# tangkk/audiomod

Measured on AMD Instinct MI355X. Metric: Msamples/s (48 kHz stereo) phase-vocoder pitch-shift; x real-time per GPU, higher is better.
Workload: dtype f32; 1 GPU; configs[1]: normal_pitchshift +4 st, stereo 48 kHz, fft=2048, phase-locked; streams_per_gpu=128, channels=2, block=480, hop_in=203, slices_per_channel=14190, concurrent_stream_groups=1, parallelism=stream-sharded x1, no collective, rank_sync=none

## Files before the change

audiomod_amd/csrc/pv_kernels.hip:

```cpp
#include "pv_kernels.h"
#include "pv_atan2f.h"
#include "pv_sincos.h"
#include "pv_wavefft.h"

#include <hip/hip_runtime.h>
#include <cstdlib>

namespace pv {

#ifdef PV_POISON
__device__ __forceinline__ void pv_poison_lds(char *base) {
    const uint32_t bytes = ((const __attribute__((address_space(4))) uint32_t *)__builtin_amdgcn_dispatch_ptr())[7];
    const int nt = blockDim.x * blockDim.y * blockDim.z, tid = threadIdx.x;
    for (uint32_t i = tid; i < bytes / 4; i += nt) reinterpret_cast<uint32_t *>(base)[i] = 0x7fc0dead;
    __syncthreads();
}
#define PV_POISON_LDS(base) pv_poison_lds(base)
#else
#define PV_POISON_LDS(base) ((void)0)
#endif

#define PV_PI 3.14159265358979323846

__device__ __forceinline__ float2 cmul(float2 a, float2 b) {
// ... 2678 lines not shown
            if (j < NP || tail_lane) acc4[q[j]] = write_back(j, V[j]);
        }
    } else {
#pragma unroll
        for (int j = 0; j < NS; ++j) asm volatile("" : "=v"(V[j].x), "=v"(V[j].y), "=v"(V[j].z), "=v"(V[j].w));
    }
    chain_pass_turn(l.turn, tl, lane);
    __builtin_amdgcn_s_setprio(0);
    float *__restrict__ out = c.out + (int64_t)row * c.out_stride_row + sl.k_off;
    float *__restrict__ stream = c.stream + (int64_t)row * ((int64_t)c.smask + 1);
    const bool quiet = (sl.flags & 2) != 0;
    auto emit = [&](int sidx, float y) {
        if (quiet || sidx < 0 || sidx >= sl.adv) return;
        if (c.resample) {
            stream[(uint32_t)(sl.str_pos + sidx) & (uint32_t)c.smask] = y;
        } else if (sidx < sl.kcnt) {
            out[sidx] = y;
        }
    };
#pragma unroll
    for (int j = 0; j < NS; ++j) {
        if (256 * j - R_ < sl.adv) {
            const int u = lane + 64 * j;
            const float4 d = j < 2 ? wd[j < 2 ? j : 0]
                                   : *reinterpret_cast<const float4 *>(wden + 4 * (u < fin_quads ? u : 0));
            const int s0 = 4 * u - R_;
            if (j < NP || tail_lane) {
                emit(s0, kFast ? V[j].x * d.x : V[j].x / d.x);
                emit(s0 + 1, kFast ? V[j].y * d.y : V[j].y / d.y);
                emit(s0 + 2, kFast ? V[j].z * d.z : V[j].z / d.z);
                emit(s0 + 3, kFast ? V[j].w * d.w : V[j].w / d.w);
            }
        }
    }
}

constexpr int chain_kernel_max_threads(int NC, int kPlainCore, bool kFast) {
    return NC <= 1024 ? ((kPlainCore < 0 || (kPlainCore == 3 && !kFast)) ? 768 : 1024) : 512;
}
template <int NC, int kPlainCore, int kRes, bool kFast = false>
__global__ __launch_bounds__(chain_kernel_max_threads(NC, kPlainCore, kFast)) void pv_synth_chain_kernel(
    const SynthArgs s, const ChainArgs c) {
    extern __shared__ __attribute__((aligned(16))) char smem_raw[];
    PV_POISON_LDS(reinterpret_cast<char *>(smem_raw));
    using W = WF<NC>;
    constexpr int N = 2 * NC, hs = NC, NQ = N / 4, NP = NQ / 64;
    const int wave = __builtin_amdgcn_readfirstlane(threadIdx.x >> 6), lane = threadIdx.x & 63;
    const int row = blockIdx.x, run = blockIdx.y;
    const int i_begin = c.run_off[run], i_count = c.run_off[run + 1] - i_begin;
    cf *wlds = reinterpret_cast<cf *>(smem_raw) + wave * W::LDS_CF;
    const ChainLds l = chain_carve(c, smem_raw + (size_t)c.waves * W::LDS_CF * sizeof(cf));
    chain_prologue(c, l, row, run == 0);
    const float *__restrict__ w = s.tb.window;
    const bool upper = (row % c.C) > 0;
    const int lane0 = lane;
    for (int i = wave; i < i_count; i += c.waves) {
        int lane = lane0;
        asm volatile("" : "+v"(lane));
        const ChainSlice sl = c.slices[i_begin + i];
        const int tl = sl.tl;
        const bool skip = (sl.flags & 1) && upper;
        float4 A[NP];
        if (!skip) {
            if (!PV_CHAIN_DIAG(c, 8)) synth_wave_role<NC, kPlainCore, 1, kFast>(s, row, tl, wlds, lane);
#pragma unroll
            for (int j = 0; j < NP; ++j) {
                const int i = 4 * (lane + 64 * j);
                const int e = ((i + hs) & (N - 1)) >> 1;
                const cf z0 = wlds[W::pad(e)], z1 = wlds[W::pad(e) + 1];
                const float4 ww = *reinterpret_cast<const float4 *>(w + i);
                A[j] = make_float4(z0.x * ww.x, z0.y * ww.y, z1.x * ww.z, z1.y * ww.w);
            }
        }
        const int r = sl.acc_pos & 3;
        if (r == 0) chain_slice_tail<0, NP, kRes, kFast>(c, l, sl, A, skip, row, i, lane);
        else if (r == 1) chain_slice_tail<1, NP, kRes, kFast>(c, l, sl, A, skip, row, i, lane);
        else if (r == 2) chain_slice_tail<2, NP, kRes, kFast>(c, l, sl, A, skip, row, i, lane);
        else chain_slice_tail<3, NP, kRes, kFast>(c, l, sl, A, skip, row, i, lane);
    }
    chain_epilogue(c, l, row, run == (int)gridDim.y - 1);
}

template <int kRes> __global__ __launch_bounds__(1024) void pv_frames_chain_kernel(const ChainArgs c) {
    extern __shared__ __attribute__((aligned(16))) char smem_raw[];
    PV_POISON_LDS(reinterpret_cast<char *>(smem_raw));
    const int wave = __builtin_amdgcn_readfirstlane(threadIdx.x >> 6), lane = threadIdx.x & 63;
    const int row = blockIdx.x, run = blockIdx.y;
    const int i_begin = c.run_off[run], i_count = c.run_off[run + 1] - i_begin;
    const ChainLds l = chain_carve(c, smem_raw);
    chain_prologue(c, l, row, run == 0);
    const int NQ = c.N >> 2;
    const int groups = (NQ + 511) >> 9;
    const bool upper = (row % c.C) > 0;
    for (int i = wave; i < i_count; i += c.waves) {
        const ChainSlice sl = c.slices[i_begin + i];
        const int tl = sl.tl;
        const bool skip = (sl.flags & 1) && upper;
        ChainPrefetch pf;
        chain_prefetch(c, sl, row, lane, pf);
        const int fslot = (int)((c.t0 + tl) & (int64_t)(c.FR - 1));
        const float4 *__restrict__ fr =
            reinterpret_cast<const float4 *>(c.frames + ((int64_t)row * c.FR + fslot) * c.N);
        auto load_group = [&](int g, float4 (&A)[8]) {
#pragma unroll
            for (int j = 0; j < 8; ++j) {
                const int u = lane + 64 * (8 * g + j);
                A[j] = (u < NQ && !skip) ? fr[u] : make_float4(0.f, 0.f, 0.f, 0.f);
            }
        };
        float4 A[8];
        load_group(0, A);
        chain_wait_turn(l.turn, i);
        if (!skip) {
            float4 prevR = make_float4(0.f, 0.f, 0.f, 0.f);
            for (int g = 0; g < groups; ++g) {
                if (g > 0) load_group(g, A);
                chain_add_dispatch<8>(l.acc, c.AR, sl.acc_pos, NQ, lane, 8 * g, A, prevR, g == groups - 1);
            }
            wave_sync();
        }
        chain_finish_slice<kRes>(c, l, sl, pf, row, i, lane);
    }
    chain_epilogue(c, l, row, run == (int)gridDim.y - 1);
}

size_t chain_lds_bytes(const ChainArgs &a, int nc_wave) {
    const size_t per_wave = nc_wave == 256    ? WF<256>::LDS_CF * sizeof(cf)
                            : nc_wave == 512  ? WF<512>::LDS_CF * sizeof(cf)
                            : nc_wave == 1024 ? WF<1024>::LDS_CF * sizeof(cf)
                            : nc_wave == 2048 ? WF<2048>::LDS_CF * sizeof(cf) : 0;
    return (size_t)a.waves * per_wave + chain_shared_bytes(a);
}

template <int NC, int kPlainCore> static void launch_synth_chain_res(const SynthArgs &s, const ChainArgs &c, hipStream_t st) {
    const size_t lds = chain_lds_bytes(c, NC);
    const bool use_fast = kPlainCore >= 0 && c.fast;
    const int kMaxThreads = use_fast ? chain_kernel_max_threads(NC, kPlainCore, true) : chain_kernel_max_threads(NC, kPlainCore, false);
    if (64 * c.waves > kMaxThreads) {
        fprintf(stderr, "audiomod_pv: fused kernel launch of %d waves exceeds its bounds (%d threads): not launched\n", c.waves, kMaxThreads);
        return;
    }
    const dim3 grid(c.rows, c.runs), block(64 * c.waves);
    static unsigned long long m0 = 0, m1 = 0, f0 = 0, f1 = 0;
    if constexpr (kPlainCore >= 0) {
        if (c.fast) {
            if (!c.resample) {
                allow_big_lds_dev(pv_synth_chain_kernel<NC, kPlainCore, 0, true>, f0);
                hipLaunchKernelGGL((pv_synth_chain_kernel<NC, kPlainCore, 0, true>), grid, block, lds, st, s, c);
            } else {
                allow_big_lds_dev(pv_synth_chain_kernel<NC, kPlainCore, 1, true>, f1);
                hipLaunchKernelGGL((pv_synth_chain_kernel<NC, kPlainCore, 1, true>), grid, block, lds, st, s, c);
            }
            return;
        }
    }
    if (!c.resample) {
        allow_big_lds_dev(pv_synth_chain_kernel<NC, kPlainCore, 0>, m0);
        hipLaunchKernelGGL((pv_synth_chain_kernel<NC, kPlainCore, 0>), grid, block, lds, st, s, c);
    } else {
        allow_big_lds_dev(pv_synth_chain_kernel<NC, kPlainCore, 1>, m1);
        hipLaunchKernelGGL((pv_synth_chain_kernel<NC, kPlainCore, 1>), grid, block, lds, st, s, c);
    }
}
bool synth_chain_has_fast(const SynthArgs &s) {
    const bool plain = !s.do_freq_comp && s.voc_band_len < 0 && !s.robotic && !s.passthru && !s.whisper &&
                       !synth_generic_only() && s.coremode >= 0 && s.coremode <= 2;
    const bool fc_locked = s.do_freq_comp && s.voc_band_len < 0 && !s.robotic && !s.passthru && !s.whisper &&
                           !synth_generic_only() && s.coremode == 1;
    return (s.tb.nc == 1024 && (plain || fc_locked)) || (s.tb.nc == 2048 && plain) ||
           ((s.tb.nc == 512 || s.tb.nc == 256) && plain);
}

void launch_synth_chain(const SynthArgs &s, const ChainArgs &c, hipStream_t st) {
    const bool plain = !s.do_freq_comp && s.voc_band_len < 0 && !s.robotic && !s.passthru && !s.whisper &&
                       !synth_generic_only() && s.coremode >= 0 && s.coremode <= 2;
    const bool fc_locked = s.do_freq_comp && s.voc_band_len < 0 && !s.robotic && !s.passthru && !s.whisper &&
                           !synth_generic_only() && s.coremode == 1;
    if (s.tb.nc == 256) {
        if (plain && s.coremode == 1) launch_synth_chain_res<256, 1>(s, c, st);
        else if (plain && s.coremode == 0) launch_synth_chain_res<256, 0>(s, c, st);
        else if (plain) launch_synth_chain_res<256, 2>(s, c, st);
        else launch_synth_chain_res<256, -1>(s, c, st);
    } else if (s.tb.nc == 512) {
        if (plain && s.coremode == 1) launch_synth_chain_res<512, 1>(s, c, st);
        else if (plain && s.coremode == 0) launch_synth_chain_res<512, 0>(s, c, st);
        else if (plain) launch_synth_chain_res<512, 2>(s, c, st);
        else launch_synth_chain_res<512, -1>(s, c, st);
    } else if (s.tb.nc == 1024) {
        if (fc_locked) launch_synth_chain_res<1024, 3>(s, c, st);
        else if (plain && s.coremode == 1) launch_synth_chain_res<1024, 1>(s, c, st);
        else if (plain && s.coremode == 0) launch_synth_chain_res<1024, 0>(s, c, st);
        else if (plain) launch_synth_chain_res<1024, 2>(s, c, st);
        else launch_synth_chain_res<1024, -1>(s, c, st);
    } else {
        if (plain && s.coremode == 1) launch_synth_chain_res<2048, 1>(s, c, st);
        else if (plain && s.coremode == 0) launch_synth_chain_res<2048, 0>(s, c, st);
        else if (plain) launch_synth_chain_res<2048, 2>(s, c, st);
        else launch_synth_chain_res<2048, -1>(s, c, st);
    }
}

void launch_frames_chain(const ChainArgs &c, hipStream_t st) {
    const size_t lds = chain_lds_bytes(c, 0);
    const dim3 grid(c.rows, c.runs), block(64 * c.waves);
    static unsigned long long m0 = 0, m1 = 0;
    if (!c.resample) {
        allow_big_lds_dev(pv_frames_chain_kernel<0>, m0);
        hipLaunchKernelGGL(pv_frames_chain_kernel<0>, grid, block, lds, st, c);
    } else {
        allow_big_lds_dev(pv_frames_chain_kernel<1>, m1);
        hipLaunchKernelGGL(pv_frames_chain_kernel<1>, grid, block, lds, st, c);
    }
}

constexpr int kResRows = 4;

template <int kRes>
__global__ __launch_bounds__(kTileOut) void pv_resample_kernel(const ResArgs a) {
    extern __shared__ __attribute__((aligned(16))) char smem_raw[];
    PV_POISON_LDS(reinterpret_cast<char *>(smem_raw));
    constexpr int NR = kResRows;
    float4 *tab4 = reinterpret_cast<float4 *>(smem_raw);
    float *stab = reinterpret_cast<float *>(smem_raw);
    float *xs = reinterpret_cast<float *>(smem_raw + a.tab_bytes);
    const int nt = blockDim.x, tid = threadIdx.x;
    const ResTile tile = a.tiles[blockIdx.x];
    const int row0 = blockIdx.y * NR, NF = a.filt_len;
    const int nr = a.rows - row0 < NR ? a.rows - row0 : NR;
    uint2 oe = make_uint2(0u, 0u);
    if (tid < tile.kcnt) oe = a.otab[(int64_t)blockIdx.x * kTileOut + tid];
    float xv[NR][2];
#pragma unroll
    for (int r = 0; r < NR; ++r) {
        const float *__restrict__ st = a.stream + (int64_t)(r < nr ? row0 + r : row0) * ((int64_t)a.smask + 1);
#pragma unroll
        for (int h = 0; h < 2; ++h) {
            const int i = tid + h * kTileOut;
            const int64_t n = tile.n_lo + i;
            xv[r][h] = (i < tile.n_cnt && n >= 0) ? st[(uint32_t)n & (uint32_t)a.smask] : 0.f;
        }
    }
    if (kRes == 2) {
        const int cnt = a.oversample * (NF + 1);
        for (int i = tid; i < cnt; i += nt) tab4[i] = a.tab4[i];
    } else {
        for (int i = tid; i < a.sinc_len; i += nt) stab[i] = a.sinc[i];
    }
#pragma unroll
    for (int r = 0; r < NR; ++r) {
#pragma unroll
        for (int h = 0; h < 2; ++h) {
            const int i = tid + h * kTileOut;
            if (i < tile.n_cnt) xs[r * a.lds_floats + i] = xv[r][h];
        }
    }
    for (int i = tid + 2 * kTileOut; i < tile.n_cnt; i += nt)
        for (int r = 0; r < nr; ++r) {
            const int64_t n = tile.n_lo + i;
            const float *__restrict__ st = a.stream + (int64_t)(row0 + r) * ((int64_t)a.smask + 1);
            xs[r * a.lds_floats + i] = n >= 0 ? st[(uint32_t)n & (uint32_t)a.smask] : 0.f;
        }
    __syncthreads();
    if (tid >= tile.kcnt) return;
    float *__restrict__ out = a.out + (int64_t)row0 * a.out_stride_row + (tile.k0 - a.k_base) + tid;
    const float *x = xs + (int)(oe.x & 0xffffu);
    if (kRes == 2) {
        const float frac = __uint_as_float(oe.y);
        const float4 *__restrict__ T = tab4 + (int)(oe.x >> 16) * (NF + 1);
        v2f a01[NR], a23[NR];
#pragma unroll
        for (int r = 0; r < NR; ++r) a01[r] = v2f{0.f, 0.f}, a23[r] = v2f{0.f, 0.f};
#pragma unroll 4
        for (int j = 0; j < NF; ++j) {
            const float4 c = T[j];
            const v2f c01 = {c.x, c.y}, c23 = {c.z, c.w};
#pragma unroll
            for (int r = 0; r < NR; ++r) {
                const float xr = x[r * a.lds_floats + j];
                const v2f xx = {xr, xr};
                a01[r] += xx * c01;
                a23[r] += xx * c23;
            }
        }
        const float c0 = -0.16667f * frac + 0.16667f * frac * frac * frac;
        const float c1 = frac + 0.5f * frac * frac - 0.5f * frac * frac * frac;
        const float c3 = -0.33333f * frac + 0.5f * frac * frac - 0.16667f * frac * frac * frac;
        const float c2 = (float)(1. - c0 - c1 - c3);
#pragma unroll
        for (int r = 0; r < NR; ++r)
            if (r < nr)
                out[(int64_t)r * a.out_stride_row] = (c0 * a01[r].x) + (c1 * a01[r].y) + (c2 * a23[r].x) + (c3 * a23[r].y);
    } else {
        const float *t = stab + (oe.x >> 16) * (uint32_t)NF;
        for (int r = 0; r < nr; ++r) {
            float sum = 0.f;
            for (int j = 0; j < NF; ++j) sum += x[r * a.lds_floats + j] * t[j];
            out[(int64_t)r * a.out_stride_row] = sum;
        }
    }
}

constexpr int kResFastRows = 16;

template <int kRes, int NR>
__global__ __launch_bounds__(kTileOut) void pv_resample_fast_kernel(const ResArgs a) {
    extern __shared__ __attribute__((aligned(16))) char smem_raw[];
    PV_POISON_LDS(reinterpret_cast<char *>(smem_raw));
    float4 *tab4 = reinterpret_cast<float4 *>(smem_raw);
    float *stab = reinterpret_cast<float *>(smem_raw);
    float *xs = reinterpret_cast<float *>(smem_raw + a.tab_bytes);
    const int nt = blockDim.x, tid = threadIdx.x;
    const ResTile tile = a.tiles[blockIdx.x];
    const int row0 = blockIdx.y * NR, NF = a.filt_len;
    const int nr = a.rows - row0 < NR ? a.rows - row0 : NR;
    uint2 oe = make_uint2(0u, 0u);
    if (tid < tile.kcnt) oe = a.otab[(int64_t)blockIdx.x * kTileOut + tid];
    for (int i = tid; i < tile.n_cnt; i += nt) {
        const int64_t n = tile.n_lo + i;
        float xv[NR];
#pragma unroll
        for (int r = 0; r < NR; ++r) {
            const float *__restrict__ st = a.stream + (int64_t)(r < nr ? row0 + r : row0) * ((int64_t)a.smask + 1);
            xv[r] = n >= 0 ? st[(uint32_t)n & (uint32_t)a.smask] : 0.f;
        }
#pragma unroll
        for (int r = 0; r < NR; ++r) xs[r * a.lds_floats + i] = xv[r];
    }
    if (kRes == 2) {
        const int cnt = a.oversample * (NF + 1);
        for (int i = tid; i < cnt; i += nt) tab4[i] = a.tab4[i];
    } else {
        for (int i = tid; i < a.sinc_len; i += nt) stab[i] = a.sinc[i];
    }
    __syncthreads();
    if (tid >= tile.kcnt) return;
    float *__restrict__ out = a.out + (int64_t)row0 * a.out_stride_row + (tile.k0 - a.k_base) + tid;
    const float *x = xs + (int)(oe.x & 0xffffu);
    float acc[NR];
#pragma unroll
    for (int r = 0; r < NR; ++r) acc[r] = 0.f;
    if (kRes == 2) {
        const float frac = __uint_as_float(oe.y);
        const float c0 = -0.16667f * frac + 0.16667f * frac * frac * frac;
        const float c1 = frac + 0.5f * frac * frac - 0.5f * frac * frac * frac;
        const float c3 = -0.33333f * frac + 0.5f * frac * frac - 0.16667f * frac * frac * frac;
        const float c2 = (float)(1. - c0 - c1 - c3);
        const float4 *__restrict__ T = tab4 + (int)(oe.x >> 16) * (NF + 1);
#pragma unroll 4
        for (int j = 0; j < NF; ++j) {
#if defined(PV_EXP_RES) && (PV_EXP_RES & 2)
            const float4 c = make_float4(frac, c0, c1, (float)j);
#else
            const float4 c = T[j];
#endif
            const float h = __builtin_fmaf(c3, c.w, __builtin_fmaf(c2, c.z, __builtin_fmaf(c1, c.y, c0 * c.x)));
#pragma unroll
            for (int r = 0; r < NR; ++r) {
#if defined(PV_EXP_RES) && (PV_EXP_RES & 1)
                acc[r] = __builtin_fmaf(frac + (float)r, h, acc[r]);
#else
                acc[r] = __builtin_fmaf(x[r * a.lds_floats + j], h, acc[r]);
#endif
            }
        }
    } else {
        const float *t = stab + (oe.x >> 16) * (uint32_t)NF;
#pragma unroll 4
        for (int j = 0; j < NF; ++j) {
            const float h = t[j];
#pragma unroll
            for (int r = 0; r < NR; ++r) acc[r] = __builtin_fmaf(x[r * a.lds_floats + j], h, acc[r]);
        }
    }
#pragma unroll
    for (int r = 0; r < NR; ++r)
        if (r < nr) out[(int64_t)r * a.out_stride_row] = acc[r];
}

template <int NR> static void launch_resample_fast_rows(const ResArgs &a, hipStream_t st) {
    const size_t lds = (size_t)a.tab_bytes + sizeof(float) * (size_t)a.lds_floats * NR;
    const dim3 grid(a.ntiles, (a.rows + NR - 1) / NR);
    static unsigned long long m1 = 0, m2 = 0;
    if (a.interp) {
        allow_big_lds_dev(pv_resample_fast_kernel<2, NR>, m2);
        hipLaunchKernelGGL((pv_resample_fast_kernel<2, NR>), grid, dim3(kTileOut), lds, st, a);
    } else {
        allow_big_lds_dev(pv_resample_fast_kernel<1, NR>, m1);
        hipLaunchKernelGGL((pv_resample_fast_kernel<1, NR>), grid, dim3(kTileOut), lds, st, a);
    }
}
static void launch_resample_fast(const ResArgs &a, hipStream_t st) {
    static const int rows_env = [] {
        const char *e = getenv("AUDIOMOD_PV_RES_ROWS");
        return e ? atoi(e) : 0;
    }();
    const int want = rows_env ? rows_env : kResFastRows;
    if (want >= 16 && a.rows >= 16 && (size_t)a.tab_bytes + sizeof(float) * (size_t)a.lds_floats * 16 <= 64 * 1024)
        launch_resample_fast_rows<16>(a, st);
    else
        launch_resample_fast_rows<8>(a, st);
}

void launch_resample(const ResArgs &a, hipStream_t st) {
    if (a.ntiles <= 0) return;
    if (a.fast) return launch_resample_fast(a, st);
    const size_t lds = (size_t)a.tab_bytes + sizeof(float) * (size_t)a.lds_floats * kResRows;
    const dim3 grid(a.ntiles, (a.rows + kResRows - 1) / kResRows);
    static unsigned long long m1 = 0, m2 = 0;
    if (a.interp) {
        allow_big_lds_dev(pv_resample_kernel<2>, m2);
        hipLaunchKernelGGL(pv_resample_kernel<2>, grid, dim3(kTileOut), lds, st, a);
    } else {
        allow_big_lds_dev(pv_resample_kernel<1>, m1);
        hipLaunchKernelGGL(pv_resample_kernel<1>, grid, dim3(kTileOut), lds, st, a);
    }
}

constexpr int kStreamThreads = 512;

__device__ __forceinline__ void stage_handoff() {
    __threadfence();
    __builtin_amdgcn_s_dcache_inv();
    __syncthreads();
}

template <int NC> __global__ __launch_bounds__(kStreamThreads) void pv_stream_kernel(const StreamArgs s) {
    extern __shared__ __attribute__((aligned(16))) char smem_raw[];
    PV_POISON_LDS(reinterpret_cast<char *>(smem_raw));
    const int wave = __builtin_amdgcn_readfirstlane(threadIdx.x >> 6), nw = kStreamThreads / 64;
    const int Tn = s.aa.Tn, rows = s.aa.rows, work = rows * Tn;
    cf *wlds = reinterpret_cast<cf *>(smem_raw) + wave * WF<NC>::LDS_CF;
    for (int i = wave; i < work; i += nw)
        analyze_wave_role<NC, (kStreamThreads / 64) * WF<NC>::LDS_CF * sizeof(cf)>(s.aa, i / Tn, i % Tn, wlds);
    stage_handoff();
    if (s.coremode == 1) {
        for (int i = wave; i < work; i += nw)
            match_wave_role(s.ma, i / Tn, i % Tn, smem_raw + (size_t)wave * match_wave_lds(s.ma.hs, s.ma.PKP));
        stage_handoff();
        for (int row = 0; row < rows; ++row) {
            seq_role<1>(s.qa, row, smem_raw);
            stage_handoff();
        }
    } else if (s.coremode == 0) {
        for (int row = 0; row < rows; ++row)
            for (int i = threadIdx.x; i < s.pa.hs; i += kStreamThreads) prop_role(s.pa, row, i);
        stage_handoff();
    }
    if (s.cepstral) {
        for (int i = wave; i < work; i += nw) cepstral_wave_role<NC>(s.ca, i / Tn, i % Tn, wlds);
        stage_handoff();
    }
    for (int i = wave; i < work; i += nw) synth_wave_role<NC>(s.sa, i / Tn, i % Tn, wlds);
    stage_handoff();
    for (int tile = 0; tile < s.oa.ntiles; ++tile)
        for (int row = 0; row < rows; ++row) {
            ola_role<1>(s.oa, tile, row, smem_raw);
            __syncthreads();
        }
}

static size_t stream_lds_bytes(const StreamArgs &s) {
    const size_t per_wave = (s.aa.tb.nc == 1024 ? WF<1024>::LDS_CF : WF<2048>::LDS_CF) * sizeof(cf);
    size_t lds = (kStreamThreads / 64) * per_wave + 4 * PV_ATAN_BLOB_WORDS;
    const size_t m = (kStreamThreads / 64) * match_wave_lds(s.ma.hs, s.ma.PKP);
    if (s.coremode == 1 && m > lds) lds = m;
    if (s.coremode == 1 && seq_lds_bytes(s.qa) > lds) lds = seq_lds_bytes(s.qa);
    if (ola_lds_bytes(s.oa, 1) > lds) lds = ola_lds_bytes(s.oa, 1);
    return lds;
}

bool stream_kernel_supported(const StreamArgs &s) {
    return (s.aa.tb.nc == 1024 || s.aa.tb.nc == 2048) && stream_lds_bytes(s) <= 160 * 1024 - 512;
}

bool lds_starts_at_zero() {
    const void *ks[] = {reinterpret_cast<const void *>(pv_analyze_wave_kernel<256, 1>),
                        reinterpret_cast<const void *>(pv_analyze_wave_kernel<512, 1>),
                        reinterpret_cast<const void *>(pv_analyze_wave_kernel<1024, 1>),
                        reinterpret_cast<const void *>(pv_analyze_wave_kernel<2048, 1>),
                        reinterpret_cast<const void *>(pv_stream_kernel<1024>),
                        reinterpret_cast<const void *>(pv_stream_kernel<2048>)};
    for (const void *k : ks) {
        hipFuncAttributes fa{};
        if (hipFuncGetAttributes(&fa, k) != hipSuccess || fa.sharedSizeBytes != 0) return false;
    }
    return true;
}

void launch_stream(const StreamArgs &s, hipStream_t st) {
    const size_t lds = stream_lds_bytes(s);
    if (s.aa.tb.nc == 1024) {
        static unsigned long long big1 = 0;
        allow_big_lds_dev(pv_stream_kernel<1024>, big1);
        hipLaunchKernelGGL((pv_stream_kernel<1024>), dim3(1), dim3(kStreamThreads), lds, st, s);
    } else {
        static unsigned long long big2 = 0;
        allow_big_lds_dev(pv_stream_kernel<2048>, big2);
        hipLaunchKernelGGL((pv_stream_kernel<2048>), dim3(1), dim3(kStreamThreads), lds, st, s);
    }
}

template <int NC, int kPlainCore, int kRes, bool kFast>
__device__ __forceinline__ void pool_synth_chain_role(const SynthArgs &s, const ChainArgs &c, const int row, char *smem_raw) {
    using W = WF<NC>;
    constexpr int N = 2 * NC, hs = NC, NQ = N / 4, NP = NQ / 64;
    const int wave = __builtin_amdgcn_readfirstlane(threadIdx.x >> 6), lane = threadIdx.x & 63;
    constexpr int run = 0;
    const int i_begin = c.run_off[run], i_count = c.run_off[run + 1] - i_begin;
    cf *wlds = reinterpret_cast<cf *>(smem_raw) + wave * W::LDS_CF;
    const ChainLds l = chain_carve(c, smem_raw + (size_t)c.waves * W::LDS_CF * sizeof(cf));
    chain_prologue(c, l, row, run == 0);
    const float *__restrict__ w = s.tb.window;
    const bool upper = (row % c.C) > 0;
    const int lane0 = lane;
    for (int i = wave; i < i_count; i += c.waves) {
        int lane = lane0;
        asm volatile("" : "+v"(lane));
        const ChainSlice sl = c.slices[i_begin + i];
        const int tl = sl.tl;
        const bool skip = (sl.flags & 1) && upper;
        float4 A[NP];
        if (!skip) {
            if (!PV_CHAIN_DIAG(c, 8)) synth_wave_role<NC, kPlainCore, 1, kFast>(s, row, tl, wlds, lane);
#pragma unroll
            for (int j = 0; j < NP; ++j) {
                const int i = 4 * (lane + 64 * j);
                const int e = ((i + hs) & (N - 1)) >> 1;
                const cf z0 = wlds[W::pad(e)], z1 = wlds[W::pad(e) + 1];
                const float4 ww = *reinterpret_cast<const float4 *>(w + i);
                A[j] = make_float4(z0.x * ww.x, z0.y * ww.y, z1.x * ww.z, z1.y * ww.w);
            }
        }
        const int r = sl.acc_pos & 3;
        if (r == 0) chain_slice_tail<0, NP, kRes, kFast>(c, l, sl, A, skip, row, i, lane);
        else if (r == 1) chain_slice_tail<1, NP, kRes, kFast>(c, l, sl, A, skip, row, i, lane);
        else if (r == 2) chain_slice_tail<2, NP, kRes, kFast>(c, l, sl, A, skip, row, i, lane);
        else chain_slice_tail<3, NP, kRes, kFast>(c, l, sl, A, skip, row, i, lane);
    }
    chain_epilogue(c, l, row, true);
}

template <int kRes>
__device__ __forceinline__ void pool_resample_role(const ResArgs &a, const unsigned tile_i, const unsigned grp, char *smem_raw) {
    constexpr int NR = kResRows;
    float4 *tab4 = reinterpret_cast<float4 *>(smem_raw);
    float *stab = reinterpret_cast<float *>(smem_raw);
    float *xs = reinterpret_cast<float *>(smem_raw + a.tab_bytes);
    const int nt = blockDim.x, tid = threadIdx.x;
    const ResTile tile = a.tiles[tile_i];
    const int row0 = grp * NR, NF = a.filt_len;
    const int nr = a.rows - row0 < NR ? a.rows - row0 : NR;
    uint2 oe = make_uint2(0u, 0u);
    if (tid < tile.kcnt) oe = a.otab[(int64_t)tile_i * kTileOut + tid];
    float xv[NR][2];
#pragma unroll
    for (int r = 0; r < NR; ++r) {
        const float *__restrict__ st = a.stream + (int64_t)(r < nr ? row0 + r : row0) * ((int64_t)a.smask + 1);
#pragma unroll
        for (int h = 0; h < 2; ++h) {
            const int i = tid + h * kTileOut;
            const int64_t n = tile.n_lo + i;
            xv[r][h] = (i < tile.n_cnt && n >= 0) ? st[(uint32_t)n & (uint32_t)a.smask] : 0.f;
        }
    }
    if (kRes == 2) {
        const int cnt = a.oversample * (NF + 1);
        for (int i = tid; i < cnt; i += nt) tab4[i] = a.tab4[i];
    } else {
        for (int i = tid; i < a.sinc_len; i += nt) stab[i] = a.sinc[i];
    }
#pragma unroll
    for (int r = 0; r < NR; ++r) {
#pragma unroll
        for (int h = 0; h < 2; ++h) {
            const int i = tid + h * kTileOut;
            if (i < tile.n_cnt) xs[r * a.lds_floats + i] = xv[r][h];
        }
    }
    for (int i = tid + 2 * kTileOut; i < tile.n_cnt; i += nt)
        for (int r = 0; r < nr; ++r) {
            const int64_t n = tile.n_lo + i;
            const float *__restrict__ st = a.stream + (int64_t)(row0 + r) * ((int64_t)a.smask + 1);
            xs[r * a.lds_floats + i] = n >= 0 ? st[(uint32_t)n & (uint32_t)a.smask] : 0.f;
        }
    __syncthreads();
    if (tid >= tile.kcnt) return;
    float *__restrict__ out = a.out + (int64_t)row0 * a.out_stride_row + (tile.k0 - a.k_base) + tid;
    const float *x = xs + (int)(oe.x & 0xffffu);
    if (kRes == 2) {
        const float frac = __uint_as_float(oe.y);
        const float4 *__restrict__ T = tab4 + (int)(oe.x >> 16) * (NF + 1);
        v2f a01[NR], a23[NR];
#pragma unroll
        for (int r = 0; r < NR; ++r) a01[r] = v2f{0.f, 0.f}, a23[r] = v2f{0.f, 0.f};
#pragma unroll 4
        for (int j = 0; j < NF; ++j) {
            const float4 c = T[j];
            const v2f c01 = {c.x, c.y}, c23 = {c.z, c.w};
#pragma unroll
            for (int r = 0; r < NR; ++r) {
                const float xr = x[r * a.lds_floats + j];
                const v2f xx = {xr, xr};
                a01[r] += xx * c01;
                a23[r] += xx * c23;
            }
        }
        const float c0 = -0.16667f * frac + 0.16667f * frac * frac * frac;
        const float c1 = frac + 0.5f * frac * frac - 0.5f * frac * frac * frac;
        const float c3 = -0.33333f * frac + 0.5f * frac * frac - 0.16667f * frac * frac * frac;
        const float c2 = (float)(1. - c0 - c1 - c3);
#pragma unroll
        for (int r = 0; r < NR; ++r)
            if (r < nr)
                out[(int64_t)r * a.out_stride_row] = (c0 * a01[r].x) + (c1 * a01[r].y) + (c2 * a23[r].x) + (c3 * a23[r].y);
    } else {
        const float *t = stab + (oe.x >> 16) * (uint32_t)NF;
        for (int r = 0; r < nr; ++r) {
            float sum = 0.f;
            for (int j = 0; j < NF; ++j) sum += x[r * a.lds_floats + j] * t[j];
            out[(int64_t)r * a.out_stride_row] = sum;
        }
    }
}

template <int kRes, int NR>
__device__ __forceinline__ void pool_resample_fast_role(const ResArgs &a, const unsigned tile_i, const unsigned grp, char *smem_raw) {
    float4 *tab4 = reinterpret_cast<float4 *>(smem_raw);
    float *stab = reinterpret_cast<float *>(smem_raw);
    float *xs = reinterpret_cast<float *>(smem_raw + a.tab_bytes);
    const int nt = blockDim.x, tid = threadIdx.x;
    const ResTile tile = a.tiles[tile_i];
    const int row0 = grp * NR, NF = a.filt_len;
    const int nr = a.rows - row0 < NR ? a.rows - row0 : NR;
    uint2 oe = make_uint2(0u, 0u);
    if (tid < tile.kcnt) oe = a.otab[(int64_t)tile_i * kTileOut + tid];
    for (int i = tid; i < tile.n_cnt; i += nt) {
        const int64_t n = tile.n_lo + i;
        float xv[NR];
#pragma unroll
        for (int r = 0; r < NR; ++r) {
            const float *__restrict__ st = a.stream + (int64_t)(r < nr ? row0 + r : row0) * ((int64_t)a.smask + 1);
            xv[r] = n >= 0 ? st[(uint32_t)n & (uint32_t)a.smask] : 0.f;
        }
#pragma unroll
        for (int r = 0; r < NR; ++r) xs[r * a.lds_floats + i] = xv[r];
    }
    if (kRes == 2) {
        const int cnt = a.oversample * (NF + 1);
        for (int i = tid; i < cnt; i += nt) tab4[i] = a.tab4[i];
    } else {
        for (int i = tid; i < a.sinc_len; i += nt) stab[i] = a.sinc[i];
    }
    __syncthreads();
    if (tid >= tile.kcnt) return;
    float *__restrict__ out = a.out + (int64_t)row0 * a.out_stride_row + (tile.k0 - a.k_base) + tid;
    const float *x = xs + (int)(oe.x & 0xffffu);
    float acc[NR];
#pragma unroll
    for (int r = 0; r < NR; ++r) acc[r] = 0.f;
    if (kRes == 2) {
        const float frac = __uint_as_float(oe.y);
        const float c0 = -0.16667f * frac + 0.16667f * frac * frac * frac;
        const float c1 = frac + 0.5f * frac * frac - 0.5f * frac * frac * frac;
        const float c3 = -0.33333f * frac + 0.5f * frac * frac - 0.16667f * frac * frac * frac;
        const float c2 = (float)(1. - c0 - c1 - c3);
        const float4 *__restrict__ T = tab4 + (int)(oe.x >> 16) * (NF + 1);
#pragma unroll 4
        for (int j = 0; j < NF; ++j) {
#if defined(PV_EXP_RES) && (PV_EXP_RES & 2)
            const float4 c = make_float4(frac, c0, c1, (float)j);
#else
            const float4 c = T[j];
#endif
            const float h = __builtin_fmaf(c3, c.w, __builtin_fmaf(c2, c.z, __builtin_fmaf(c1, c.y, c0 * c.x)));
#pragma unroll
            for (int r = 0; r < NR; ++r) {
#if defined(PV_EXP_RES) && (PV_EXP_RES & 1)
                acc[r] = __builtin_fmaf(frac + (float)r, h, acc[r]);
#else
                acc[r] = __builtin_fmaf(x[r * a.lds_floats + j], h, acc[r]);
#endif
            }
        }
    } else {
        const float *t = stab + (oe.x >> 16) * (uint32_t)NF;
#pragma unroll 4
        for (int j = 0; j < NF; ++j) {
            const float h = t[j];
#pragma unroll
            for (int r = 0; r < NR; ++r) acc[r] = __builtin_fmaf(x[r * a.lds_floats + j], h, acc[r]);
        }
    }
#pragma unroll
    for (int r = 0; r < NR; ++r)
        if (r < nr) out[(int64_t)r * a.out_stride_row] = acc[r];
}

__global__ __launch_bounds__(256) void pv_pool_ingest_kernel(const float *__restrict__ src, float *__restrict__ ring,
// ... 584 lines not shown
```

Before: 16650 Msamples/s.

## Add MFMA-based resampler kernel using 16x16x4 f32 matrix ops

Adds a new resample kernel that computes the polyphase FIR over 16 rows and 16 outputs per wave with MFMA f32 16x16x4 instructions instead of per-thread scalar FMAs. Samples are staged in LDS with a padded stride. Filter taps are built per lane and zeroed outside the window. Non-finite inputs trigger a fallback to the VALU path, which is factored into a shared helper. The MFMA path is on by default, can be disabled via an env var, and adds padding work and per-step clamping overhead.

```diff
diff --git a/audiomod_amd/csrc/pv_kernels.hip b/audiomod_amd/csrc/pv_kernels.hip
--- a/audiomod_amd/csrc/pv_kernels.hip
+++ b/audiomod_amd/csrc/pv_kernels.hip
@@ -3004,6 +3004,61 @@
 
 constexpr int kResFastRows = 16;
 
+__device__ __forceinline__ float4 res_cubic_coef(const float frac) {
+    const float c0 = -0.16667f * frac + 0.16667f * frac * frac * frac;
+    const float c1 = frac + 0.5f * frac * frac - 0.5f * frac * frac * frac;
+    const float c3 = -0.33333f * frac + 0.5f * frac * frac - 0.16667f * frac * frac * frac;
+    const float c2 = (float)(1. - c0 - c1 - c3);
+    return make_float4(c0, c1, c2, c3);
+}
+__device__ __forceinline__ float res_cubic_tap(const float4 c, const float4 t) {
+    return __builtin_fmaf(c.w, t.w, __builtin_fmaf(c.z, t.z, __builtin_fmaf(c.y, t.y, c.x * t.x)));
+}
+
+template <int kRes, int NR>
+__device__ __forceinline__ void res_fast_valu(const ResArgs &a, const uint2 oe, const float *xs, const int xstride,
+                                              const int nrl, const float4 *tab4, const float *stab,
+                                              float *__restrict__ out, const int nr) {
+    const int NF = a.filt_len;
+    const float *x = xs + (int)(oe.x & 0xffffu);
+    float acc[NR];
+#pragma unroll
+    for (int r = 0; r < NR; ++r) acc[r] = 0.f;
+    if (kRes == 2) {
+        const float frac = __uint_as_float(oe.y);
+        const float4 cw = res_cubic_coef(frac);
+        const float4 *__restrict__ T = tab4 + (int)(oe.x >> 16) * (NF + 1);
+#pragma unroll 4
+        for (int j = 0; j < NF; ++j) {
+#if defined(PV_EXP_RES) && (PV_EXP_RES & 2)
+            const float4 c = make_float4(frac, cw.x, cw.y, (float)j);
+#else
+            const float4 c = T[j];
+#endif
+            const float h = res_cubic_tap(cw, c);
+#pragma unroll
+            for (int r = 0; r < NR; ++r) {
+#if defined(PV_EXP_RES) && (PV_EXP_RES & 1)
+                acc[r] = __builtin_fmaf(frac + (float)r, h, acc[r]);
+#else
+                acc[r] = __builtin_fmaf(x[(r < nrl ? r : 0) * xstride + j], h, acc[r]);
+#endif
+            }
+        }
+    } else {
+        const float *t = stab + (oe.x >> 16) * (uint32_t)NF;
+#pragma unroll 4
+        for (int j = 0; j < NF; ++j) {
+            const float h = t[j];
+#pragma unroll
+            for (int r = 0; r < NR; ++r) acc[r] = __builtin_fmaf(x[(r < nrl ? r : 0) * xstride + j], h, acc[r]);
+        }
+    }
+#pragma unroll
+    for (int r = 0; r < NR; ++r)
+        if (r < nr) out[(int64_t)r * a.out_stride_row] = acc[r];
+}
+
 template <int kRes, int NR>
 __global__ __launch_bounds__(kTileOut) void pv_resample_fast_kernel(const ResArgs a) {
     extern __shared__ __attribute__((aligned(16))) char smem_raw[];
@@ -3037,46 +3092,138 @@
     __syncthreads();
     if (tid >= tile.kcnt) return;
     float *__restrict__ out = a.out + (int64_t)row0 * a.out_stride_row + (tile.k0 - a.k_base) + tid;
-    const float *x = xs + (int)(oe.x & 0xffffu);
-    float acc[NR];
-#pragma unroll
-    for (int r = 0; r < NR; ++r) acc[r] = 0.f;
+    res_fast_valu<kRes, NR>(a, oe, xs, a.lds_floats, NR, tab4, stab, out, nr);
+}
+
+constexpr int kResMfmaRows = 16;
+constexpr int kResMfmaBlocks = 4;
+
+typedef float v4f __attribute__((ext_vector_type(4)));
+
+__host__ __device__ constexpr int res_mfma_xstride(const int lds_floats) { return ((lds_floats - 2) & ~3) + 2; }
+
+template <int kRes>
+__global__ __launch_bounds__(kTileOut) __attribute__((amdgpu_waves_per_eu(4))) void pv_resample_mfma_kernel(const ResArgs a) {
+    extern __shared__ __attribute__((aligned(16))) char smem_raw[];
+    PV_POISON_LDS(reinterpret_cast<char *>(smem_raw));
+    constexpr int NR = kResMfmaRows, NW = kTileOut / 64, NB = kResMfmaBlocks, NBW = kTileOut / 16 / NW;
+    const float4 *tab4 = reinterpret_cast<const float4 *>(smem_raw);
+    const float *stab = reinterpret_cast<const float *>(smem_raw);
+    float *xs = reinterpret_cast<float *>(smem_raw + a.tab_bytes);
+    const int tid = threadIdx.x, lane = tid & 63, w = tid >> 6;
+    const ResTile tile = a.tiles[blockIdx.x];
+    const int row0 = blockIdx.y * NR, NF = a.filt_len, ncnt = tile.n_cnt, kcnt = tile.kcnt;
+    const int nr = a.rows - row0 < NR ? a.rows - row0 : NR;
+    const int nrl = a.rows < NR ? a.rows : NR;
+    const bool fits = ncnt + 4 <= res_mfma_xstride(a.lds_floats);
+    const int xstride = fits ? res_mfma_xstride(a.lds_floats) : a.lds_floats;
+    const int nstage = fits ? ncnt + 4 : ncnt;
+    const uint2 *__restrict__ ot = a.otab + (int64_t)blockIdx.x * kTileOut;
+    const int q = lane >> 4, c = lane & 15;
+    uint2 eo[NBW];
+#pragma unroll
+    for (int k = 0; k < NBW; ++k) {
+        const int n = 16 * (w + NW * k) + c;
+        eo[k] = n < kcnt ? ot[n] : make_uint2(0u, 0u);
+    }
+    bool bad = false;
+    for (int i = tid; i < nstage; i += kTileOut) {
+        const int64_t n = tile.n_lo + i;
+        float xv[NR];
+#pragma unroll
+        for (int r = 0; r < NR; ++r) {
+            const float *__restrict__ st = a.stream + (int64_t)(row0 + r) * ((int64_t)a.smask + 1);
+            xv[r] = (r < nr && i < ncnt && n >= 0) ? st[(uint32_t)n & (uint32_t)a.smask] : 0.f;
+        }
+#pragma unroll
+        for (int r = 0; r < NR; ++r)
+            if (r < nr) {
+                xs[r * xstride + i] = xv[r];
+                bad |= (__float_as_uint(xv[r]) & 0x7f800000u) == 0x7f800000u;
+            }
+    }
     if (kRes == 2) {
-        const float frac = __uint_as_float(oe.y);
-        const float c0 = -0.16667f * frac + 0.16667f * frac * frac * frac;
-        const float c1 = frac + 0.5f * frac * frac - 0.5f * frac * frac * frac;
-        const float c3 = -0.33333f * frac + 0.5f * frac * frac - 0.16667f * frac * frac * frac;
-        const float c2 = (float)(1. - c0 - c1 - c3);
-        const float4 *__restrict__ T = tab4 + (int)(oe.x >> 16) * (NF + 1);
-#pragma unroll 4
-        for (int j = 0; j < NF; ++j) {
-#if defined(PV_EXP_RES) && (PV_EXP_RES & 2)
-            const float4 c = make_float4(frac, c0, c1, (float)j);
-#else
-            const float4 c = T[j];
+        const int cnt = a.oversample * (NF + 1);
+        for (int i = tid; i < cnt; i += kTileOut) reinterpret_cast<float4 *>(smem_raw)[i] = a.tab4[i];
+    } else {
+        for (int i = tid; i < a.sinc_len; i += kTileOut) reinterpret_cast<float *>(smem_raw)[i] = a.sinc[i];
+    }
+    int *flag = reinterpret_cast<int *>(xs + nrl * xstride);
+    const bool wave_bad = __any(bad);
+    if (fits && lane == 0) flag[w] = wave_bad ? 1 : 0;
+    __syncthreads();
+    bool vec = !fits;
+    if (fits) {
+#pragma unroll
+        for (int i = 0; i < NW; ++i) vec |= flag[i] != 0;
+    }
+    float *__restrict__ out = a.out + (int64_t)row0 * a.out_stride_row + (tile.k0 - a.k_base);
+    if (vec) {
+        if (tid < kcnt) res_fast_valu<kRes, NR>(a, ot[tid], xs, xstride, nr, tab4, stab, out + tid, nr);
+        return;
+    }
+    const float *xa = xs + (c < nr ? c : 0) * xstride + q;
+#pragma unroll 1
+    for (int p = 0; p < NBW / NB; ++p) {
+        int base[NB], jb[NB], nk[NB], nb[NB];
+        float4 cw[NB];
+        const float4 *T[NB];
+        const float *S[NB];
+        int ks = 0;
+#pragma unroll
+        for (int b = 0; b < NB; ++b) {
+            const int n0 = 16 * (w + NW * (p * NB + b));
+            const int n = n0 + c;
+            const uint2 e = eo[p * NB + b];
+            const int off = (int)(e.x & 0xffffu);
+            const int last = (kcnt - 1 - n0 < 15 ? kcnt - 1 - n0 : 15);
+            base[b] = __builtin_amdgcn_readfirstlane(off);
+            nk[b] = last < 0 ? 0 : (__builtin_amdgcn_readlane(off, last < 0 ? 0 : last) - base[b] + NF + 3) >> 2;
+            ks = nk[b] > ks ? nk[b] : ks;
+            jb[b] = n < kcnt ? q - (off - base[b]) : -(1 << 29);
+            nb[b] = n0;
+            if constexpr (kRes == 2) {
+                cw[b] = res_cubic_coef(__uint_as_float(e.y));
+                T[b] = tab4 + (int)(e.x >> 16) * (NF + 1);
+            } else {
+                S[b] = stab + (e.x >> 16) * (uint32_t)NF;
+            }
+        }
+        ks = __builtin_amdgcn_readfirstlane(ks);
+        if (ks == 0) break;
+        v4f acc[NB];
+#pragma unroll
+        for (int b = 0; b < NB; ++b) acc[b] = v4f{0.f, 0.f, 0.f, 0.f};
+        auto step = [&](const int s) {
+#pragma unroll
+            for (int b = 0; b < NB; ++b) {
+                const uint32_t j = (uint32_t)(jb[b] + 4 * s), jc = j < (uint32_t)(NF - 1) ? j : (uint32_t)(NF - 1);
+                float h;
+                if constexpr (kRes == 2) h = res_cubic_tap(cw[b], T[b][jc]);
+                else h = S[b][jc];
+                h = j < (uint32_t)NF ? h : 0.f;
+                const int t = base[b] + 4 * s < ncnt ? base[b] + 4 * s : ncnt;
+                acc[b] = __builtin_amdgcn_mfma_f32_16x16x4f32(xa[t], h, acc[b], 0, 0, 0);
+            }
+        };
+        int s = 0;
+#if defined(PV_EXP_RES) && (PV_EXP_RES & 4)
+        s = ks;
 #endif
-            const float h = __builtin_fmaf(c3, c.w, __builtin_fmaf(c2, c.z, __builtin_fmaf(c1, c.y, c0 * c.x)));
-#pragma unroll
-            for (int r = 0; r < NR; ++r) {
-#if defined(PV_EXP_RES) && (PV_EXP_RES & 1)
-                acc[r] = __builtin_fmaf(frac + (float)r, h, acc[r]);
-#else
-                acc[r] = __builtin_fmaf(x[r * a.lds_floats + j], h, acc[r]);
-#endif
-            }
-        }
-    } else {
-        const float *t = stab + (oe.x >> 16) * (uint32_t)NF;
-#pragma unroll 4
-        for (int j = 0; j < NF; ++j) {
-            const float h = t[j];
-#pragma unroll
-            for (int r = 0; r < NR; ++r) acc[r] = __builtin_fmaf(x[r * a.lds_floats + j], h, acc[r]);
-        }
-    }
-#pragma unroll
-    for (int r = 0; r < NR; ++r)
-        if (r < nr) out[(int64_t)r * a.out_stride_row] = acc[r];
+#pragma unroll 1
+        for (; s + 4 <= ks; s += 4) step(s), step(s + 1), step(s + 2), step(s + 3);
+#pragma unroll 1
+        for (; s < ks; ++s) step(s);
+#pragma unroll
+        for (int b = 0; b < NB; ++b) {
+            const int n = nb[b] + c;
+            if (n < kcnt) {
+#pragma unroll
+                for (int i = 0; i < 4; ++i)
+                    if (4 * q + i < nr) out[(int64_t)(4 * q + i) * a.out_stride_row + n] = acc[b][i];
+            }
+        }
+    }
 }
 
 template <int NR> static void launch_resample_fast_rows(const ResArgs &a, hipStream_t st) {
@@ -3096,6 +3243,26 @@
         const char *e = getenv("AUDIOMOD_PV_RES_ROWS");
         return e ? atoi(e) : 0;
     }();
+    static const bool mfma = [] {
+        const char *e = getenv("AUDIOMOD_PV_RES_MFMA");
+        return !(e && atoi(e) == 0);
+    }();
+    const size_t fl = sizeof(float);
+    if (mfma && (size_t)a.tab_bytes + fl * (size_t)a.lds_floats * kResMfmaRows <= 64 * 1024) {
+        const size_t nrl = a.rows < kResMfmaRows ? a.rows : kResMfmaRows;
+        const size_t padded = fl * (nrl * res_mfma_xstride(a.lds_floats) + kTileOut / 64);
+        const size_t lds = (size_t)a.tab_bytes + std::max(fl * nrl * (size_t)a.lds_floats, padded);
+        const dim3 grid(a.ntiles, (a.rows + kResMfmaRows - 1) / kResMfmaRows);
+        static unsigned long long m1 = 0, m2 = 0;
+        if (a.interp) {
+            allow_big_lds_dev(pv_resample_mfma_kernel<2>, m2);
+            hipLaunchKernelGGL(pv_resample_mfma_kernel<2>, grid, dim3(kTileOut), lds, st, a);
+        } else {
+            allow_big_lds_dev(pv_resample_mfma_kernel<1>, m1);
+            hipLaunchKernelGGL(pv_resample_mfma_kernel<1>, grid, dim3(kTileOut), lds, st, a);
+        }
+        return;
+    }
     const int want = rows_env ? rows_env : kResFastRows;
     if (want >= 16 && a.rows >= 16 && (size_t)a.tab_bytes + sizeof(float) * (size_t)a.lds_floats * 16 <= 64 * 1024)
         launch_resample_fast_rows<16>(a, st);
```

After: 17170 Msamples/s, median of 6. 3.1% higher.
